# uga-ssrl/SSRLCV

Hardware: AMD Instinct MI355X
Metric: Mpix/s SIFT extract (+ Mmatches/s 128-D brute-force, see `matcher`) (higher is better)
Workload: dtype f32; 1 GPU; 2-view 4096x4096 pair per GPU (tools/scene.py pinhole views (PCG32 terrain + texture through Image::Camera)): SIFT_FeatureFactory::generateFeatures (sparse DoG path) on each image, pixels resident in HBM; images_per_gpu=2, parallelism=image-pair shard, library=release build (libssrlcv_hip_release.so)

## Files before the change

ssrlcv_amd/csrc/dev_switch.h:

```cpp
#pragma once
#include <stddef.h>
#include <stdint.h>
#include <stdlib.h>

#if (defined(SSRLCV_STAMPS) || defined(SSRLCV_MATCH_STATS) || defined(SSRLCV_TIMING_VARIANT)) && !defined(SSRLCV_INSTRUMENTED_BUILD)
#error "SSRLCV_STAMPS / SSRLCV_MATCH_STATS only build through `make instrumented` or the tools/ lab programs (-DSSRLCV_INSTRUMENTED_BUILD)"
#endif
#if defined(SSRLCV_LAB) || defined(SSRLCV_MATCH_LAB) || defined(SSRLCV_LAB_LOCAL_GATHER) || defined(SSRLCV_LAB_UPS_LOADS)
#error "the timing-lab variants (results invalid) were removed in round 6; see git history before 2026-10-05"
#endif

#ifndef SSRLCV_THETAS_LANES_SHIFT
#define SSRLCV_THETAS_LANES_SHIFT 2
#endif
#ifndef SSRLCV_PAIR_F32_MINPX
#define SSRLCV_PAIR_F32_MINPX (~(size_t)0)
#endif
static_assert(SSRLCV_THETAS_LANES_SHIFT >= 0 && SSRLCV_THETAS_LANES_SHIFT <= 2, "k_thetas is built for 1, 2 or 4 lanes per key point");

namespace svdev __attribute__((visibility("hidden"))) {
#ifdef SSRLCV_RELEASE
constexpr bool flag(const char*) { return false; }
constexpr int integer(const char*, int unset) { return unset; }
constexpr size_t size(const char*, size_t unset) { return unset; }
constexpr float real(const char*, float unset) { return unset; }
constexpr char first_char(const char*) { return 0; }
#else
inline const char* env(const char* name) { return getenv(name); }
inline bool flag(const char* name) { return env(name) != nullptr; }
inline int integer(const char* name, int unset) { return env(name) ? atoi(env(name)) : unset; }
inline size_t size(const char* name, size_t unset) { return env(name) ? (size_t)atoll(env(name)) : unset; }
inline float real(const char* name, float unset) { return env(name) ? (float)atof(env(name)) : unset; }
inline char first_char(const char* name) { return env(name) ? env(name)[0] : 0; }
#endif
template <typename T>
constexpr T positive_or(T v, T otherwise) { return v > 0 ? v : otherwise; }
constexpr int one_or_two(int n) { return n == 1 || n == 2 ? n : 0; }
constexpr int lanes_to_shift(int lanes) { return lanes >= 4 ? 2 : (lanes >= 2 ? 1 : 0); }

struct Switches {
  bool gaussValu = flag("SSRLCV_GAUSS_VALU");
  bool gaussMfma = flag("SSRLCV_GAUSS_MFMA");
  bool gaussWide = flag("SSRLCV_GAUSS_WIDE");
  bool gaussNarrow = flag("SSRLCV_GAUSS_NARROW");
  int gaussMfmaMinR = integer("SSRLCV_GAUSS_MFMA_MINR", 11);
  size_t gaussTileMaxPx = size("SSRLCV_GAUSS_TILE_MAXPX", (size_t)1 << 20);
  int gaussRm = integer("SSRLCV_GAUSS_RM", 4 | 8 | 16);
  size_t gaussRmMinPx = size("SSRLCV_GAUSS_RM_MINPX", (size_t)1 << 24);
  int gaussRmOneb = integer("SSRLCV_GAUSS_RM_ONEB", 0);
  int gaussRmRows = integer("SSRLCV_GAUSS_RM_ROWS", 0);
  bool noGaussPair = flag("SSRLCV_NO_GAUSS_PAIR");
  bool noGaussPairRm = flag("SSRLCV_NO_GAUSS_PAIR_RM");
  size_t gaussPairMinPx = size("SSRLCV_GAUSS_PAIR_MINPX", (size_t)1 << 26);
  size_t gaussPairMinPxF32 = size("SSRLCV_GAUSS_PAIR_MINPX_F32", SSRLCV_PAIR_F32_MINPX);
  bool gaussPairValuForm = first_char("SSRLCV_GAUSS_PAIR_FORM") == 'v';
  int pairRows = integer("SSRLCV_PAIR_ROWS", 0);
  bool noUpsampleFusion = flag("SSRLCV_NO_UPSAMPLE_FUSION");
  bool noBinFusion = flag("SSRLCV_NO_BIN_FUSION");
  bool noXcdStrips = flag("SSRLCV_NO_XCD_STRIPS");
  int dogxNpx = integer("SSRLCV_DOGX_NPX", 0);
  int dogSplit = integer("SSRLCV_DOG_SPLIT", 0) != 0 ? 1 : 0;
  unsigned dogxWaves = positive_or((unsigned)integer("SSRLCV_DOGX_WAVES", 0), 14336u);
  int dogx0After = one_or_two(integer("SSRLCV_DOGX0_AFTER", 0));
  bool noOctaveOverlap = flag("SSRLCV_NO_OCTAVE_OVERLAP");
  int octaveOverlapFrom = integer("SSRLCV_OCTAVE_OVERLAP_FROM", 1);
  int phased = integer("SSRLCV_PHASED", 0);
  bool earlyPolar = flag("SSRLCV_EARLY_POLAR");
  bool noEarlyChain = flag("SSRLCV_NO_EARLY_CHAIN");
  bool siftSerial = flag("SSRLCV_SIFT_SERIAL");
  int prio = integer("SSRLCV_PRIO", 0);
  bool sideLowPriority = flag("SSRLCV_SIDE_LOW_PRIORITY");
  int thetasLanesShift = lanes_to_shift(integer("SSRLCV_THETAS_LANES", 1 << SSRLCV_THETAS_LANES_SHIFT));
  bool thetasSplit = flag("SSRLCV_THETAS_SPLIT");
  bool samplingPipelined = flag("SSRLCV_SAMPLING_PIPELINED");
  bool samplingIrregular = flag("SSRLCV_SAMPLING_IRREGULAR");
  bool stagedGlue = (prio & 4) != 0;
#if defined(SSRLCV_INSTRUMENTED_BUILD) && !defined(SSRLCV_RELEASE)
  uint32_t timingThetasSel = env("SSRLCV_TIMING_THETAS_SEL") ? (uint32_t)strtoul(env("SSRLCV_TIMING_THETAS_SEL"), nullptr, 16) : 0xFFFFFu;
#else
  uint32_t timingThetasSel = 0xFFFFFu;
#endif
  bool matchF16 = flag("SSRLCV_MATCH_F16");
  float bandDir = real("SSRLCV_BAND_DIR", 1e30f);
  float bandStrip = real("SSRLCV_BAND_STRIP", 0.0f);
  float bandStripQ = real("SSRLCV_BAND_STRIP_Q", 0.0f);
  int mergeThreads = positive_or(integer("SSRLCV_MERGE_THREADS", 1), 1);
  bool mergeTiming = flag("SSRLCV_MERGE_TIMING");
};

#ifdef SSRLCV_RELEASE
constexpr Switches kDefaults{};
constexpr const Switches& sw() { return kDefaults; }
#else
inline Switches& sw() {
  static Switches s;
  return s;
}
#endif
}
```

ssrlcv_amd/csrc/keypoints.hip:

```cpp
#include <hip/hip_runtime.h>
#include <float.h>
#include <math.h>
#include <stdlib.h>
#include "compact.h"
#include "dev_switch.h"
#include "scan_lookback.h"
#include "device_math.h"
#include "sift_plan.h"
#include "ssrlcv_hip.h"

using svp::OctaveState;

namespace {

struct LevelSet {
  const float* lvl[svp::kGauss];
  const float* lvlMinMax;
  const float* minmax;
  const float2* polar;
  int w, h;
};

struct DogView {
  const float* lo;
// ... 393 lines not shown
        const int lo = st[o].idx[seg], hi = seg < svp::kDog - 1 ? st[o].idx[seg + 1] : st[o].n;
        if (hi > lo) { first = (uint32_t)lo; count = (uint32_t)(hi - lo); }
      }
      tab->first[r] = first;
      tab->count[r] = count;
      tab->start[r] = pos;
      pos += (count + (1u << unitShift) - 1) >> unitShift;
    }
  }
  tab->total = pos;
}
__global__ void k_build_ranges(const OctaveState* st, RangeTable* tab, int unitShift, uint32_t sel) { build_ranges(st, tab, unitShift, sel); }
__global__ void k_book_and_desc_ranges(OctaveState* st, uint32_t* featBase, uint32_t* numFeatures, uint32_t maxFeatures, RangeTable* tab) {
  uint32_t tot = 0;
  for (int o = 0; o < svp::kOctaves; ++o) {
    featBase[o] = tot;
    tot += st[o].hasExtrema ? (uint32_t)st[o].n : 0u;
  }
  if (tot > maxFeatures) tot = maxFeatures;
  *numFeatures = tot;
  build_ranges(st, tab, 0, 0xFFFFFu);
}

constexpr int kOct0Groups = svp::kSampleGroups - 1;
struct GroupCtl {
  uint32_t segStart[svp::kDog];
  uint32_t totals[svp::kSampleGroups + 1];
  uint32_t groupSum[svp::kSampleGroups];
  uint32_t done[svp::kSampleGroups];
  uint32_t regular;
  uint32_t cut[2];
  uint32_t pad[32 - svp::kDog - 3 * svp::kSampleGroups - 4];
};
static_assert(sizeof(GroupCtl) == 128, "four of them + eight range tables fit the plan's 4 KB group block");
__device__ __forceinline__ bool blur_indices_regular(const OctaveState* st) {
  if (!st->hasExtrema) return true;
  bool ok = st->idx[0] == 0;
  for (int k = 1; k < svp::kDog; ++k) ok = ok && st->idx[k - 1] <= st->idx[k];
  return ok && st->idx[svp::kDog - 1] <= st->n;
}
__global__ void k_build_group_ranges(const OctaveState* st, RangeTable* tabs, GroupCtl* ctl, int unitShift, bool forceIrregular) {
  const bool reg = blur_indices_regular(st) && !forceIrregular;
  const uint32_t n0 = st[0].hasExtrema && st[0].n > 0 ? (uint32_t)st[0].n : 0u;
  ctl[0].regular = reg ? 1u : 0u;
  ctl[0].cut[0] = reg && n0 ? (uint32_t)st[0].idx[2] : n0;
  ctl[0].cut[1] = reg && n0 ? (uint32_t)st[0].idx[3] : n0;
  const uint32_t oct0 = 0x1Fu, rest = 0xFFFFFu & ~oct0;
  build_ranges(st, tabs + 0, unitShift, reg ? 0x03u : oct0);
  build_ranges(st, tabs + 1, unitShift, reg ? 0x04u : 0u);
  build_ranges(st, tabs + 2, unitShift, reg ? 0x18u : 0u);
  build_ranges(st, tabs + 3, unitShift, rest);
}
__global__ void k_build_desc_ranges_oct0(const OctaveState* st, RangeTable* tab, const GroupCtl* ctl, int g, uint32_t cap) {
  if (!ctl->regular) {
    build_ranges(st, tab, 0, g == kOct0Groups - 1 ? 0x1Fu : 0u);
    return;
  }
  const int segLo = g == 0 ? 0 : g + 1, segHi = g == 0 ? 2 : (g == 1 ? 3 : svp::kDog);
  const uint32_t end = ctl->totals[g + 1] < cap ? ctl->totals[g + 1] : cap;
  auto start_of = [&](int seg) {
    if (seg >= segHi) return end;
    const uint32_t enc = ctl->segStart[seg];
    const uint32_t v = enc ? enc - 1u : end;
    return v < end ? v : end;
  };
  uint32_t pos = 0;
  for (int k = 0; k < 5; ++k) {
    const int seg = kSegOrder[k];
    for (int o = 0; o < svp::kOctaves; ++o) {
      const int r = k * 4 + o;
      uint32_t first = 0, count = 0;
      if (o == 0 && seg >= segLo && seg < segHi) {
        const uint32_t lo = start_of(seg), hi = start_of(seg + 1);
        if (hi > lo) { first = lo; count = hi - lo; }
      }
      tab->first[r] = first;
      tab->count[r] = count;
      tab->start[r] = pos;
      pos += count;
    }
  }
  tab->total = pos;
}
__device__ __forceinline__ int range_of(const RangeTable* tab, uint32_t u) {
  int r = 0;
#pragma unroll
  for (int k = 1; k < 20; ++k)
    if (tab->start[k] <= u) r = k;
  return r;
}

struct OctaveSet {
  LevelSet L[svp::kOctaves];
  const ssrlcv_sskeypoint* kps[svp::kOctaves];
  float pixelWidth[svp::kOctaves];
  float* thetas[svp::kOctaves];
  uint32_t* thetaCnt[svp::kOctaves];
  const void* consts[svp::kOctaves];
};

template <int MAXO, int LPKS>
__global__ __launch_bounds__(64) void k_thetas(const OctaveState* states, const RangeTable* tab, OctaveSet set, float lambda,
                                               float orientationThreshold) {
  constexpr int LANES = 1 << LPKS, PER_BLOCK = 64 >> LPKS, CW = kThetaChunk * LANES;
  __shared__ float s_hist[36][PER_BLOCK];
  if (blockIdx.x >= tab->total) return;
  const int range = __builtin_amdgcn_readfirstlane(range_of(tab, blockIdx.x));
  const int octave = range & 3, useg = kSegOrder[range >> 2];
  const LevelSet& L = set.L[octave];
  const float pixelWidth = set.pixelWidth[octave];
  const int t = threadIdx.x, sub = t & (LANES - 1), col = t >> LPKS;
  const float fsub2 = (float)(2 * sub);
  const uint32_t local = (blockIdx.x - tab->start[range]) * PER_BLOCK + (uint32_t)(t >> LPKS);
  const bool have = local < tab->count[range];
  const int gi = (int)(tab->first[range] + local);
  const float pi = SSRLCV_PI_F;
  const float rad10 = pi / 18.0f;
  const float inv10 = 1.0f / rad10;
  ssrlcv_sskeypoint kp;
  kp.loc.x = kp.loc.y = 0.0f;
  kp.sigma = 1.0f;
  if (have) kp = set.kps[octave][gi];
  const float kx = kp.loc.x, ky = kp.loc.y;
  const float windowWidth = ceilf(kp.sigma * 3.0f * lambda / pixelWidth);
  const float minx = kx - windowWidth, miny = ky - windowWidth, maxx = kx + windowWidth, maxy = ky + windowWidth;
  const bool inside = have && useg >= 1 && useg <= 3 &&
                      !(minx < 0.0f || miny < 0.0f || maxx >= (unsigned)(L.w - 1) || maxy >= (unsigned)(L.h - 1));
#pragma unroll
  for (int i = 0; i < 36 * PER_BLOCK / 64; ++i) (&s_hist[0][0])[i * 64 + t] = 0.0f;
  const float weight = 2.0f * lambda * lambda * kp.sigma * kp.sigma;
  const float rweight = 1.0f / weight;
  const int W = L.w;
  const size_t levelStride = svp::polar_level_stride(L.w, L.h);
  {
    const float2* base = L.polar + (size_t)(useg - 1) * levelStride;
    const __amdgpu_buffer_rsrc_t rsrc = __builtin_amdgcn_make_buffer_rsrc((void*)base, 0, (int)(uint32_t)(levelStride * 8), 0x00020000);
    typedef unsigned u32x4 __attribute__((ext_vector_type(4)));
    typedef unsigned u32x2 __attribute__((ext_vector_type(2)));
    struct Cursor { float x, y, ty2; unsigned rowoff; bool act; };
    Cursor cf;
    cf.x = minx;
    cf.y = miny;
    cf.ty2 = (miny - ky) * (miny - ky);
    cf.rowoff = (unsigned)round_pos(miny) * (unsigned)W + 1u;
    cf.act = inside;
    auto advance = [&](Cursor& c) {
      float xn = c.x + (float)CW;
      if (__any(c.act && !(c.x >= (float)CW))) {
        float ch = c.x;
#pragma unroll 8
        for (int i = 0; i < CW; ++i) ch += 1.0f;
        xn = c.x >= (float)CW ? xn : ch;
      }
      if (c.act) {
        if (xn <= maxx) {
          c.x = xn;
        } else {
          c.x = minx;
          c.y += 1.0f;
          if (!(c.y <= maxy)) c.act = false;
          const float ty = c.y - ky;
          c.ty2 = ty * ty;
          c.rowoff = (unsigned)round_pos(c.y) * (unsigned)W + 1u;
        }
      }
    };
    typedef u32x4 Chunk[kThetaChunk / 2];
// ... 91 lines not shown
              const float n1 = fmaf(mg[2 * j + 1], wg[2 * j + 1], slot[2 * j + 1] == slot[2 * j] ? n0 : h1);
              *slot[2 * j] = n0;
              *slot[2 * j + 1] = n1;
            }
            if (LANES > 1) __builtin_amdgcn_wave_barrier();
          }
        }
      };
      weigh_half(std::integral_constant<int, 0>{});
      if (upperHalf) weigh_half(std::integral_constant<int, 1>{});
      vote_half(std::integral_constant<int, 0>{});
      if (upperHalf) vote_half(std::integral_constant<int, 1>{});
    };
    while (__any(ca.act)) {
      step(qa, ca, qb, cb);
      if (!__any(cb.act)) break;
      step(qb, cb, qa, ca);
    }
  }
  uint32_t cnt = 0;
  float outTheta[MAXO];
#pragma unroll
  for (int i = 0; i < MAXO; ++i) outTheta[i] = -FLT_MAX;
  if (inside && sub == 0) {
    float maxHist = 0.0f;
    for (int i = 0; i < 36; ++i) {
      const float h = s_hist[i][col];
      if (h > maxHist) maxHist = h;
    }
    maxHist *= orientationThreshold;
    float bestMag[MAXO], bestTh[MAXO];
#pragma unroll
    for (int i = 0; i < MAXO; ++i) { bestMag[i] = 0.0f; bestTh[i] = 0.0f; }
    float hprev = s_hist[35][col], hb = s_hist[0][col];
    for (int b = 0; b < 36; ++b) {
      const float hnext = s_hist[b == 35 ? 0 : b + 1][col];
      if (!(hb < maxHist || hb < hprev || hb < hnext || hb < bestMag[MAXO - 1])) {
        float tmag = hb;
        float tt = (hprev - hnext) / (hprev - (2.0f * hb) + hnext);
        tt *= (pi / 36.0f);
        tt += (b * rad10);
        tt = fmodf(tt + (2.0f * pi), 2.0f * pi);
#pragma unroll
        for (int i = 0; i < MAXO; ++i) {
          if (tmag > bestMag[i]) {
#pragma unroll
            for (int ii = i; ii < MAXO; ++ii) {
              float m2 = bestMag[ii], t2 = bestTh[ii];
              bestMag[ii] = tmag;
              bestTh[ii] = tt;
              tmag = m2;
              tt = t2;
            }
          }
        }
      }
      hprev = hb;
      hb = hnext;
    }
#pragma unroll
    for (int i = 0; i < MAXO; ++i) {
      if (bestMag[i] != 0.0f) { outTheta[i] = bestTh[i]; cnt = i + 1; }
    }
  }
  if (have && sub == 0) {
#pragma unroll
    for (int i = 0; i < MAXO; ++i) set.thetas[octave][(size_t)gi * svp::kMaxOrient + i] = outTheta[i];
    set.thetaCnt[octave][gi] = cnt;
  }
}

__device__ __forceinline__ float uniform_f(float v) {
  return __builtin_bit_cast(float, __builtin_amdgcn_readfirstlane(__builtin_bit_cast(int, v)));
}
struct DescConst {
  float c, s;
  float windowWidth;
  float invExpDen;
  float voteScale;
  float invBin;
  uint32_t magic;
  int32_t segment;
};
static_assert(sizeof(DescConst) == 32, "one s_load_dwordx8");
__global__ __launch_bounds__(256) void k_desc_consts(const RangeTable* tab, OctaveSet set, float lambda, const OctaveState* states,
                                                     const GroupCtl* regularCtl) {
  const uint32_t total = tab->total;
  const bool fromTable = regularCtl != nullptr && regularCtl->regular != 0u;
  for (uint32_t u = blockIdx.x * 256 + threadIdx.x; u < total; u += gridDim.x * 256) {
    const int range = range_of(tab, u);
    const int octave = range & 3;
    const int i = (int)(tab->first[range] + (u - tab->start[range]));
    const ssrlcv_sskeypoint* kps = set.kps[octave];
    const float pixelWidth = set.pixelWidth[octave];
    DescConst* __restrict__ out = (DescConst*)const_cast<void*>(set.consts[octave]);
    DescConst d;
    const float theta = kps[i].theta;
    d.c = sv_cosf(-theta);
    d.s = sv_sinf(-theta);
    d.windowWidth = ceilf(kps[i].sigma * lambda / pixelWidth);
    d.invExpDen = 1.0f / (2.0f * d.windowWidth * d.windowWidth);
    int boundExp;
    (void)frexpf(1.4143f * ((d.windowWidth + 2.0f) * (d.windowWidth + 2.0f)), &boundExp);
    d.voteScale = ldexpf(1.0f, 31 - boundExp);
    d.invBin = 1.0f / (d.windowWidth / 2.0f);
    const unsigned wi = (unsigned)(int)d.windowWidth;
    d.magic = wi > 1u ? 0xFFFFFFFFu / wi + 1u : 0u;
    d.segment = fromTable ? kSegOrder[range >> 2] : segment_of(states + octave, i);
    out[i] = d;
  }
}

__device__ __forceinline__ unsigned vote_u32(float v) {
  int r;
  asm("v_cvt_rpi_i32_f32 %0, %1" : "=v"(r) : "v"(v));
  return (unsigned)r;
}

#ifndef SSRLCV_DESC_COPIES
#define SSRLCV_DESC_COPIES 8
#endif
constexpr int kDescCopies = SSRLCV_DESC_COPIES;
#ifndef SSRLCV_DESC_VGPRS
#define SSRLCV_DESC_VGPRS 64
#endif
__global__ __launch_bounds__(256) __attribute__((amdgpu_waves_per_eu(4, 8), amdgpu_num_vgpr(SSRLCV_DESC_VGPRS), amdgpu_num_sgpr(102))) void k_descriptors(const RangeTable* tab, OctaveSet set, const uint32_t* featBase,
                                                     ssrlcv_sift_feature* __restrict__ features, uint32_t maxFeatures) {
  __shared__ unsigned s_bins[4][(1 + 128 + 2) * kDescCopies];
  __shared__ __attribute__((aligned(8))) uint8_t s_bytes[4][128];
  const int lane = threadIdx.x & 63, wave = __builtin_amdgcn_readfirstlane(threadIdx.x >> 6);
  unsigned* bins = s_bins[wave] + kDescCopies;
  const int copy = lane & (kDescCopies - 1);
  const float pi = SSRLCV_PI_F;
  const float rad45 = pi / 4.0f;
  const float inv45 = 1.0f / rad45;
  const uint32_t totalUnits = tab->total;
  for (uint32_t unit = blockIdx.x * 4 + wave; unit < totalUnits; unit += gridDim.x * 4) {
    const int range = range_of(tab, unit);
    const int octave = range & 3;
    const int gi = (int)(tab->first[range] + (unit - tab->start[range]));
    const LevelSet& L = set.L[octave];
    const float pixelWidth = set.pixelWidth[octave];
    const float2* __restrict__ polar = L.polar;
    const DescConst dc = reinterpret_cast<const DescConst*>(set.consts[octave])[gi];
    const ssrlcv_sskeypoint kp = set.kps[octave][gi];
    const int seg = dc.segment;
    const float kx = kp.loc.x, ky = kp.loc.y;
    const float theta = kp.theta;
    const float windowWidth = dc.windowWidth;
    const float binWidth = windowWidth / 2.0f;
    const float c = dc.c, s = dc.s;
    const float2* __restrict__ pl = polar + (size_t)(seg - 1) * svp::polar_level_stride(L.w, L.h) + 1;
#pragma unroll
    for (int i = 0; i < 2 * kDescCopies; ++i) bins[i * 64 + lane] = 0u;
    f32x2 rc[16];
    {
      const int ci = lane & 15;
      const float hx = ((float)(ci >> 2) * 0.5f - 0.75f) * windowWidth, hy = ((float)(ci & 3) * 0.5f - 0.75f) * windowWidth;
      const float rx = (hx * c) + (hy * s), ry = (-hx * s) + (hy * c);
#pragma unroll
      for (int cell = 0; cell < 16; ++cell) {
        if ((cell >> 2) == 0 || (cell & 3) == 0) continue;
        rc[cell].x = __builtin_bit_cast(float, __builtin_amdgcn_readlane(__builtin_bit_cast(int, rx), cell));
        rc[cell].y = __builtin_bit_cast(float, __builtin_amdgcn_readlane(__builtin_bit_cast(int, ry), cell));
      }
    }
    const float expDen = 2.0f * windowWidth * windowWidth, invExpDen = dc.invExpDen, invBin = dc.invBin;
    const float voteScale = dc.voteScale;
    const int Wi = (int)windowWidth;
    const unsigned centreIdx = (unsigned)(Wi * (Wi + 1));
    const unsigned magic = dc.magic;
    auto sample = [&](unsigned idx, float& cx, float& cy, bool& ok) {
      const unsigned yq = Wi == 1 ? idx : __umulhi(idx, magic);
      const unsigned xq = idx - yq * (unsigned)Wi + 1u;
      const bool centre = idx >= centreIdx;
      const float x = centre ? 0.0f : (float)(int)xq;
      const float y = centre ? 0.0f : (float)(int)yq;
      cx = (x * c) + (y * s);
      cy = (-x * s) + (y * c);
      ok = idx <= centreIdx && fmaxf(fabsf(cx), fabsf(cy)) <= windowWidth;
    };
    auto gather = [&](float px, float py) { return polar_px(pl, L.w, round_coord(px), round_coord(py)); };
    auto split = [&](float2 pg, bool live, float& w0, float& w1, unsigned*& pa, float& ang, bool& odd) {
      ang = fmod_2pi_above(pg.y - theta + (2.0f * pi), 2.0f * pi);
      const float t45 = ang * inv45;
      const float fk = floorf(t45);
      const float u = t45 - fk;
      odd = live && !(u > 1.0e-4f && u < 0.9999f);
      int k0 = (int)fk;
      const float a0 = fabsf(ang - (fk * rad45)), a1 = fabsf(ang - ((fk + 1.0f) * rad45));
      w0 = (live && !odd && (unsigned)k0 < 8u) ? 1.0f - sv::exact_div3(a0, rad45, inv45) : 0.0f;
      w1 = (live && !odd && (unsigned)(k0 + 1) < 8u) ? 1.0f - sv::exact_div3(a1, rad45, inv45) : 0.0f;
      k0 = k0 < -1 ? -1 : k0;
      pa = bins + k0 * kDescCopies + copy;
    };
    float ncx, ncy;
    bool nok;
    sample((unsigned)lane, ncx, ncy, nok);
    float2 npg[4] = {make_float2(0.0f, 0.0f), make_float2(0.0f, 0.0f), make_float2(0.0f, 0.0f), make_float2(0.0f, 0.0f)};
    auto gather4 = [&]() {
      npg[0] = gather(ncx + kx, ncy + ky);
      npg[1] = gather(kx - ncy, ncx + ky);
      npg[2] = gather(kx - ncx, ky - ncy);
      npg[3] = gather(ncy + kx, ky - ncx);
    };
    if (nok) gather4();
    for (unsigned base = 0; base <= centreIdx; base += 64) {
      const float cx = ncx, cy = ncy;
      const bool ok = nok;
      const float2 pg0 = npg[0], pg1 = npg[1], pg2 = npg[2], pg3 = npg[3];
      const bool turned = ok && base + (unsigned)lane < centreIdx;
      sample(base + 64 + (unsigned)lane, ncx, ncy, nok);
      if (nok) gather4();
      const float r2n = -((cx * cx) + (cy * cy));
      const float g = sv::expf_nonpos(sv::exact_div3(r2n, expDen, invExpDen)) * voteScale;
      float a0, a1, b0, b1, c0, c1, d0, d1, angA, angB, angC, angD;
      bool oddA, oddB, oddC, oddD;
      unsigned *pa, *pb, *pc, *pd;
      split(pg0, ok, a0, a1, pa, angA, oddA);
      split(pg1, turned, b0, b1, pb, angB, oddB);
      split(pg2, turned, c0, c1, pc, angC, oddC);
      split(pg3, turned, d0, d1, pd, angD, oddD);
      const float magA = pg0.x * g, magB = pg1.x * g, magC = pg2.x * g, magD = pg3.x * g;
      const float bwl = ok ? binWidth : -1.0f;
#pragma unroll
      for (int cell = 0; cell < 16; ++cell) {
        const int nx = cell >> 2, ny = cell & 3;
        if (nx == 0 || ny == 0) continue;
        const int cellB = (3 - ny) * 4 + nx, cellC = 15 - cell, cellD = ny * 4 + (3 - nx);
        const float tx = fabsf(rc[cell].x - cx), ty = fabsf(rc[cell].y - cy);
        if (fmaxf(tx, ty) <= bwl) {
          const float wxy = (1.0f - sv::exact_div3(tx, binWidth, invBin)) * (1.0f - sv::exact_div3(ty, binWidth, invBin));
          atomicAdd(pa + cell * 8 * kDescCopies, vote_u32((wxy * a0) * magA));
          atomicAdd(pa + cell * 8 * kDescCopies + kDescCopies, vote_u32((wxy * a1) * magA));
          atomicAdd(pb + cellB * 8 * kDescCopies, vote_u32((wxy * b0) * magB));
          atomicAdd(pb + cellB * 8 * kDescCopies + kDescCopies, vote_u32((wxy * b1) * magB));
          atomicAdd(pc + cellC * 8 * kDescCopies, vote_u32((wxy * c0) * magC));
          atomicAdd(pc + cellC * 8 * kDescCopies + kDescCopies, vote_u32((wxy * c1) * magC));
          atomicAdd(pd + cellD * 8 * kDescCopies, vote_u32((wxy * d0) * magD));
          atomicAdd(pd + cellD * 8 * kDescCopies + kDescCopies, vote_u32((wxy * d1) * magD));
        }
      }
      if (__ballot(oddA || oddB || oddC || oddD) != 0ull) {
#pragma unroll 1
        for (int m = 0; m < 4; ++m) {
          const bool odd = m == 0 ? oddA : m == 1 ? oddB : m == 2 ? oddC : oddD;
          if (!odd) continue;
          const float mcx = m == 0 ? cx : m == 1 ? -cy : m == 2 ? -cx : cy;
          const float mcy = m == 0 ? cy : m == 1 ? cx : m == 2 ? -cy : -cx;
          const float mang = m == 0 ? angA : m == 1 ? angB : m == 2 ? angC : angD;
          const float mmag = m == 0 ? magA : m == 1 ? magB : m == 2 ? magC : magD;
#pragma unroll 1
          for (int cell = 0; cell < 16; ++cell) {
            const int ci = lane & 15;
            (void)ci;
            const float hx0 = ((float)(cell >> 2) * 0.5f - 0.75f) * windowWidth, hy0 = ((float)(cell & 3) * 0.5f - 0.75f) * windowWidth;
            const float rx = (hx0 * c) + (hy0 * s), ry = (-hx0 * s) + (hy0 * c);
            float hx = fabsf(rx - mcx), hy = fabsf(ry - mcy);
            if (hx <= binWidth && hy <= binWidth) {
              hx = hx / binWidth;
              hy = hy / binWidth;
              for (int k = 0; k < 8; ++k) {
                float angle = fabsf(mang - ((float)k * rad45));
                if (angle < rad45) {
                  angle /= rad45;
                  const float temp = (1.0f - hx) * (1.0f - hy) * (1.0f - angle) * mmag;
                  atomicAdd(bins + (cell * 8 + k) * kDescCopies + copy, vote_u32(temp));
                }
              }
            }
          }
        }
      }
    }
    __builtin_amdgcn_wave_barrier();
    unsigned t0 = 0u, t1 = 0u;
#pragma unroll
    for (int cpy = 0; cpy < kDescCopies; ++cpy) {
      t0 += bins[lane * kDescCopies + cpy];
      t1 += bins[(lane + 64) * kDescCopies + cpy];
    }
    float v0 = (float)t0, v1 = (float)t1;
    float sq = sqrtf(sv::wave_sum((v0 * v0) + (v1 * v1)));
    v0 = v0 / sq;
    v1 = v1 / sq;
    if (v0 > 0.2f) v0 = 0.2f;
    if (v1 > 0.2f) v1 = 0.2f;
    sq = sqrtf(sv::wave_sum((v0 * v0) + (v1 * v1)));
    {
      int b0 = lane, b1 = lane + 64;
      int o0 = (((b0 >> 3) & 3) * 4 + (b0 >> 5)) * 8 + (b0 & 7);
      int o1 = (((b1 >> 3) & 3) * 4 + (b1 >> 5)) * 8 + (b1 & 7);
      s_bytes[wave][o0] = (uint8_t)roundf(255.0f * v0 / sq);
      s_bytes[wave][o1] = (uint8_t)roundf(255.0f * v1 / sq);
    }
    __builtin_amdgcn_wave_barrier();
    const uint32_t fi = featBase[octave] + (uint32_t)gi;
    if (fi < maxFeatures) {
      ssrlcv_sift_feature* f = features + fi;
      if (lane < 16) *reinterpret_cast<uint2*>(&f->values[lane * 8]) = *reinterpret_cast<const uint2*>(&s_bytes[wave][lane * 8]);
      if (lane == 16) {
        f->parent = -1;
        reinterpret_cast<int*>(f)[1] = 0;
        f->theta = kp.theta;
        f->sigma = kp.sigma;
        f->loc.x = kp.loc.x * pixelWidth;
        f->loc.y = kp.loc.y * pixelWidth;
      }
    }
    __builtin_amdgcn_wave_barrier();
  }
}

LevelSet make_levels(const ssrlcv_sift_plan* plan, char* ws, int o) {
  LevelSet L;
  const svp::OctavePlan& oc = plan->oct[o];
  for (int b = 0; b < svp::kGauss; ++b) L.lvl[b] = (const float*)(ws + plan->off_gauss[o][b]);
  L.lvlMinMax = (const float*)(ws + plan->off_minmax) + (size_t)o * 2 * (svp::kGauss + svp::kDog);
  L.minmax = L.lvlMinMax + 2 * svp::kGauss;
  L.polar = (const float2*)(ws + oc.off_polar);
  L.w = (int)oc.w;
  L.h = (int)oc.h;
  return L;
}

void launch_polar(const ssrlcv_sift_plan* plan, char* ws, hipStream_t st, int oFirst = 0, int oLast = svp::kOctaves - 1) {
  PolarJobs jobs;
  uint32_t pos = 0;
  for (int o = 0; o < svp::kOctaves; ++o) {
    const svp::OctavePlan& oc = plan->oct[o];
    jobs.L[o] = make_levels(plan, ws, o);
    jobs.out[o] = (float2*)(ws + oc.off_polar);
    jobs.start[o] = pos;
    jobs.tilesX[o] = (oc.w + 255) / 256;
    if (o >= oFirst && o <= oLast) pos += jobs.tilesX[o] * ((oc.h + kPolRows - 1) / kPolRows);
  }
  jobs.start[svp::kOctaves] = pos;
  hipLaunchKernelGGL(k_polar, dim3(pos), dim3(256), 0, st, jobs);
}

}
namespace svp {
void launch_polar_octave(const ssrlcv_sift_plan* plan, char* ws, int octave, hipStream_t st) {
  PolarJobs jobs;
  const svp::OctavePlan& oc = plan->oct[octave];
  const uint32_t tilesX = (oc.w + 255) / 256, tiles = tilesX * ((oc.h + kPolRows - 1) / kPolRows);
  for (int o = 0; o < svp::kOctaves; ++o) {
    jobs.L[o] = make_levels(plan, ws, octave);
    jobs.out[o] = (float2*)(ws + oc.off_polar);
    jobs.tilesX[o] = tilesX;
    jobs.start[o] = o <= octave ? 0u : tiles;
  }
  jobs.start[svp::kOctaves] = tiles;
  hipLaunchKernelGGL(k_polar, dim3(tiles), dim3(256), 0, st, jobs);
}
}
namespace {
hipError_t run_discard(OctaveState* st, const ssrlcv_sskeypoint* src, ssrlcv_sskeypoint* dst, uint32_t cap,
                       uint32_t* words, hipStream_t stream) {
  const OctaveState* cst = st;
  auto keyfn = [=] __device__(uint32_t i) -> uint32_t {
    if (!cst->hasExtrema || (int)i >= cst->n) return 0u;
    if (src[i].discard) return 0u;
    return 1u << segment_of(cst, (int)i);
  };
  auto emit = [=] __device__(uint32_t i, int, uint32_t d) { dst[d] = src[i]; };
  uint32_t* totals = nullptr;
  auto post = [=] __device__(const uint32_t* tot) { book_discard(st, tot); };
  return svc::partition<svp::kDog, 8>(cap, keyfn, emit, words, &totals, stream, &st->n, 1u, post);
}

constexpr unsigned kWaveKernelOversubscription = 16;
inline unsigned list_blocks(uint32_t cap) {
  unsigned b = (cap + 255) / 256;
  return b > 1024 ? 1024 : b;
}

}

extern "C" {

int ssrlcv_sift_plan_keypoints(const ssrlcv_sift_plan* plan, void* workspace, int octave, ssrlcv_sskeypoint** list,
                               int** blurIndices_dev) {
  if (!plan || !workspace || octave < 0 || octave >= svp::kOctaves) return SSRLCV_ERR_INVALID_ARG;
  char* ws = (char*)workspace;
  if (list) *list = (ssrlcv_sskeypoint*)(ws + (plan->listInB[octave] ? plan->oct[octave].off_kpB : plan->oct[octave].off_kpA));
  if (blurIndices_dev) *blurIndices_dev = (int*)(ws + plan->off_state + sizeof(OctaveState) * octave);
  return SSRLCV_OK;
}

// ... 415 lines not shown
  }
  return SSRLCV_OK;
}

int stage_orientations(const ssrlcv_sift_plan* plan, char* ws, uint32_t* numFeatures, hipStream_t caller, svp::PlanAsync* as, bool polarDone,
                       bool restInFlight = false, bool prologueDone = false) {
  OctaveState* states = (OctaveState*)(ws + plan->off_state);
  const uint32_t maxO = plan->params.maxOrientations;
  OctaveSet set = make_set(plan, ws);
  RangeTable* thetaRanges = theta_tab(plan, ws, 0);
  const uint32_t thetaSel = svdev::sw().timingThetasSel;
  const int lanesShift = svdev::sw().thetasLanesShift;
  const float lambdaO = plan->params.orientationContribWidth, othr = plan->params.orientationThreshold;
  if (restInFlight) {
    hipLaunchKernelGGL(k_build_ranges, dim3(1), dim3(1), 0, caller, states, thetaRanges, 6 - lanesShift, 0x1Fu & thetaSel);
    launch_thetas(maxO, lanesShift, thetas_grid(plan, 0, 0, lanesShift), caller, (const OctaveState*)states, (const RangeTable*)thetaRanges, set,
                  lambdaO, othr);
    int rc = launch_expand(plan, ws, 0, 0, 1, caller);
    if (rc) return rc;
    plan->listInB[0] ^= 1;
    SSRLCV_HIP_TRY(hipStreamWaitEvent(caller, as->expandJoin[1], 0));
    return SSRLCV_OK;
  }
  if (!svdev::sw().stagedGlue) {
    if (!prologueDone) launch_orient_prologue(plan, ws, caller);
    if (!polarDone) launch_polar(plan, ws, caller);
    launch_thetas(maxO, lanesShift, thetas_grid(plan, 0, svp::kOctaves - 1, lanesShift), caller, (const OctaveState*)states, (const RangeTable*)thetaRanges, set, lambdaO, othr);
    launch_expand_all(plan, ws, numFeatures, caller);
    for (int o = 0; o < svp::kOctaves; ++o) plan->listInB[o] ^= 1;
    return SSRLCV_OK;
  }
  if (!prologueDone) {
    const int rc = orientations_prologue(plan, ws, caller, as);
    if (rc) return rc;
  }
  if (!polarDone) launch_polar(plan, ws, caller);
  launch_thetas(maxO, lanesShift, thetas_grid(plan, 0, svp::kOctaves - 1, lanesShift), caller, (const OctaveState*)states, (const RangeTable*)thetaRanges, set, lambdaO, othr);
  if (as) {
    SSRLCV_HIP_TRY(hipEventRecord(as->groupFork, caller));
    for (int o = 1; o < svp::kOctaves; ++o) SSRLCV_HIP_TRY(hipStreamWaitEvent(expand_stream(as, caller, o), as->groupFork, 0));
  }
  for (int o = 0; o < svp::kOctaves; ++o) {
    int rc = launch_expand(plan, ws, o, 0, 1, expand_stream(as, caller, o), true);
    if (rc) return rc;
    plan->listInB[o] ^= 1;
  }
  if (as) {
    for (int o = 1; o < svp::kOctaves; ++o) {
      SSRLCV_HIP_TRY(hipEventRecord(as->groupExpanded[o - 1], expand_stream(as, caller, o)));
      SSRLCV_HIP_TRY(hipStreamWaitEvent(caller, as->groupExpanded[o - 1], 0));
    }
  }
  return SSRLCV_OK;
}

void book_features(const ssrlcv_sift_plan* plan, char* ws, uint32_t* numFeatures, hipStream_t caller, bool withDescRanges = false) {
  if (withDescRanges)
    hipLaunchKernelGGL(k_book_and_desc_ranges, dim3(1), dim3(1), 0, caller, (OctaveState*)(ws + plan->off_state),
                       (uint32_t*)(ws + plan->oct[0].off_featBase), numFeatures, plan->maxFeatures, desc_tab(plan, ws, 0));
  else
    hipLaunchKernelGGL(k_book_featbase, dim3(1), dim3(1), 0, caller, (OctaveState*)(ws + plan->off_state),
                       (uint32_t*)(ws + plan->oct[0].off_featBase), numFeatures, plan->maxFeatures);
}

unsigned desc_blocks(const ssrlcv_sift_plan* plan, int oFirst, int oLast, unsigned* maxBlocks) {
  unsigned blocks = 0, mx = 1;
  for (int o = oFirst; o <= oLast; ++o) {
    blocks += list_blocks(plan->oct[o].cap);
    mx = list_blocks(plan->oct[o].cap) > mx ? list_blocks(plan->oct[o].cap) : mx;
  }
  if (maxBlocks) *maxBlocks = mx;
  return blocks;
}

int stage_descriptors(const ssrlcv_sift_plan* plan, char* ws, ssrlcv_sift_feature* features, hipStream_t caller, bool rangesBuilt = false) {
  OctaveState* states = (OctaveState*)(ws + plan->off_state);
  OctaveSet set = make_set(plan, ws);
  RangeTable* descRanges = desc_tab(plan, ws, 0);
  uint32_t* featBase = (uint32_t*)(ws + plan->oct[0].off_featBase);
  unsigned maxBlocks = 1;
  const unsigned descBlocks = desc_blocks(plan, 0, svp::kOctaves - 1, &maxBlocks);
  if (!rangesBuilt) hipLaunchKernelGGL(k_build_ranges, dim3(1), dim3(1), 0, caller, states, descRanges, 0, 0xFFFFFu);
  hipLaunchKernelGGL(k_desc_consts, dim3(maxBlocks * svp::kOctaves), dim3(256), 0, caller, (const RangeTable*)descRanges, set,
                     plan->params.descriptorContribWidth, (const OctaveState*)states, (const GroupCtl*)nullptr);
  hipLaunchKernelGGL(k_descriptors, dim3(descBlocks * kWaveKernelOversubscription), dim3(256), 0, caller, (const RangeTable*)descRanges, set,
                     (const uint32_t*)featBase, features, plan->maxFeatures);
  return SSRLCV_OK;
}

int stage_sampling_pipelined(const ssrlcv_sift_plan* plan, char* ws, ssrlcv_sift_feature* features, uint32_t* numFeatures,
                             hipStream_t caller, svp::PlanAsync* as) {
  OctaveState* states = (OctaveState*)(ws + plan->off_state);
  const uint32_t maxO = plan->params.maxOrientations;
  const float lambdaO = plan->params.orientationContribWidth, othr = plan->params.orientationThreshold;
  const float lambdaD = plan->params.descriptorContribWidth;
  uint32_t* featBase = (uint32_t*)(ws + plan->oct[0].off_featBase);
  OctaveSet setT = make_set(plan, ws);
  for (int o = 0; o < svp::kOctaves; ++o) plan->listInB[o] ^= 1;
  OctaveSet setD = make_set(plan, ws);
  for (int o = 0; o < svp::kOctaves; ++o) plan->listInB[o] ^= 1;
  const hipStream_t gs[svp::kSampleGroups] = {caller, as->chain, as->chain2, as->table};
  const int lanesShift = svdev::sw().thetasLanesShift;
  unsigned thetaBlocks[svp::kSampleGroups], descBlocks[svp::kSampleGroups], constBlocks[svp::kSampleGroups];
  for (int g = 0; g < svp::kSampleGroups; ++g) {
    const int oFirst = g < kOct0Groups ? 0 : 1, oLast = g < kOct0Groups ? 0 : svp::kOctaves - 1;
    thetaBlocks[g] = thetas_grid(plan, oFirst, oLast, lanesShift);
    unsigned mx = 1;
    descBlocks[g] = desc_blocks(plan, oFirst, oLast, &mx) * kWaveKernelOversubscription;
    constBlocks[g] = mx * (unsigned)(oLast - oFirst + 1);
  }
  SSRLCV_HIP_TRY(hipMemsetAsync(group_ctl(plan, ws, 0), 0, sizeof(GroupCtl) * svp::kOctaves, caller));
  SSRLCV_HIP_TRY(hipMemsetAsync(featBase, 0, 4 * svp::kOctaves, caller));
  const bool forceIrregular = svdev::sw().samplingIrregular;
  hipLaunchKernelGGL(k_build_group_ranges, dim3(1), dim3(1), 0, caller, (const OctaveState*)states, theta_tab(plan, ws, 0), group_ctl(plan, ws, 0), 6 - lanesShift,
                     forceIrregular);
  SSRLCV_HIP_TRY(hipEventRecord(as->groupFork, caller));
  for (int g = 1; g < svp::kSampleGroups; ++g) SSRLCV_HIP_TRY(hipStreamWaitEvent(gs[g], as->groupFork, 0));
  for (int g = 0; g < svp::kSampleGroups; ++g)
    launch_thetas(maxO, lanesShift, thetaBlocks[g], gs[g], (const OctaveState*)states, (const RangeTable*)theta_tab(plan, ws, g), setT, lambdaO, othr);
  for (int g = 0; g < kOct0Groups; ++g) {
    if (g > 0) SSRLCV_HIP_TRY(hipStreamWaitEvent(gs[g], as->groupExpanded[g - 1], 0));
    int rc = launch_expand(plan, ws, 0, g, kOct0Groups, gs[g]);
    if (rc) return rc;
    SSRLCV_HIP_TRY(hipEventRecord(as->groupExpanded[g], gs[g]));
    hipLaunchKernelGGL(k_build_desc_ranges_oct0, dim3(1), dim3(1), 0, gs[g], (const OctaveState*)states, desc_tab(plan, ws, g),
                       (const GroupCtl*)group_ctl(plan, ws, 0), g, plan->oct[0].cap);
    hipLaunchKernelGGL(k_desc_consts, dim3(constBlocks[g]), dim3(256), 0, gs[g], (const RangeTable*)desc_tab(plan, ws, g), setD, lambdaD,
                       (const OctaveState*)states, (const GroupCtl*)group_ctl(plan, ws, 0));
    if (g > 0) SSRLCV_HIP_TRY(hipEventRecord(as->groupReady[g], gs[g]));
  }
  {
    const int g = svp::kSampleGroups - 1;
    for (int o = 1; o < svp::kOctaves; ++o) {
      int rc = launch_expand(plan, ws, o, 0, 1, gs[g]);
      if (rc) return rc;
    }
    SSRLCV_HIP_TRY(hipStreamWaitEvent(gs[g], as->groupExpanded[kOct0Groups - 1], 0));
    book_features(plan, ws, numFeatures, gs[g]);
    hipLaunchKernelGGL(k_build_ranges, dim3(1), dim3(1), 0, gs[g], (const OctaveState*)states, desc_tab(plan, ws, g), 0, 0xFFFFFu & ~0x1Fu);
    hipLaunchKernelGGL(k_desc_consts, dim3(constBlocks[g]), dim3(256), 0, gs[g], (const RangeTable*)desc_tab(plan, ws, g), setD, lambdaD,
                       (const OctaveState*)states, (const GroupCtl*)nullptr);
    SSRLCV_HIP_TRY(hipEventRecord(as->groupReady[g], gs[g]));
  }
  for (int o = 0; o < svp::kOctaves; ++o) plan->listInB[o] ^= 1;
  for (int g = 0; g < svp::kSampleGroups; ++g) {
    if (g > 0) SSRLCV_HIP_TRY(hipStreamWaitEvent(caller, as->groupReady[g], 0));
    hipLaunchKernelGGL(k_descriptors, dim3(descBlocks[g]), dim3(256), 0, caller, (const RangeTable*)desc_tab(plan, ws, g), setD,
                       (const uint32_t*)featBase, features, plan->maxFeatures);
  }
  return SSRLCV_OK;
}

int run_list_chain(const ssrlcv_sift_plan* plan, char* ws, int o, hipStream_t s) {
  const int stop = plan->stopStage;
  const ListCtx c = make_ctx(plan, ws, o, s);
  int rc = stage_extrema(c, stop >= 1);
  if (!rc && stop >= 2) rc = stage_refine(c);
  if (!rc && stop >= 5) rc = stage_noise_edges_window(c);
  else {
    if (!rc && stop >= 3) rc = stage_noise(c, svp::kNoiseThreshold);
    if (!rc && stop >= 4) rc = stage_edges(c);
  }
  return rc;
}

}
namespace svp {
int launch_chain_octave(const ssrlcv_sift_plan* plan, char* ws, int octave, hipStream_t st) { return run_list_chain(plan, ws, octave, st); }
}
extern "C" {

static void drain_side_streams(const ssrlcv_sift_plan* plan, hipStream_t st) {
  svp::PlanAsync* as = plan->asyncState == 1 ? plan->async : nullptr;
  if (as) {
    for (hipStream_t side : {as->chain, as->table, as->chain2, as->polar}) {
      if (hipEventRecord(as->fork, side) == hipSuccess) (void)hipStreamWaitEvent(st, as->fork, 0);
    }
    (void)hipGetLastError();
  }
  plan->chain0InFlight = 0;
  plan->polarInFlight = 0;
}
static int describe_impl(const ssrlcv_sift_plan* plan, void* workspace, ssrlcv_sift_feature* features, uint32_t* numFeatures, ssrlcv_stream_t stream);
int ssrlcv_hip_sift_describe(const ssrlcv_sift_plan* plan, void* workspace, ssrlcv_sift_feature* features, uint32_t* numFeatures,
                             ssrlcv_stream_t stream) {
  const int rc = describe_impl(plan, workspace, features, numFeatures, stream);
  if (rc && plan) drain_side_streams(plan, (hipStream_t)stream);
  return rc;
}
static int describe_impl(const ssrlcv_sift_plan* plan, void* workspace, ssrlcv_sift_feature* features,
                             uint32_t* numFeatures, ssrlcv_stream_t stream) {
  if (!plan || !workspace || !numFeatures) return SSRLCV_ERR_INVALID_ARG;
  char* ws = (char*)workspace;
  const int stop = plan->stopStage;
  if (stop >= 7 && !features) return SSRLCV_ERR_INVALID_ARG;
  svp::PlanAsync* as = svp::plan_async(plan);
  const hipStream_t caller = (hipStream_t)stream;
  const bool splitWanted = svdev::sw().thetasSplit, pipelinedSampling = svdev::sw().samplingPipelined;
  const bool splitRest = as && stop >= 6 && !plan->polarInFlight && splitWanted && !pipelinedSampling;
  if (splitRest) SSRLCV_HIP_TRY(hipMemsetAsync(group_ctl(plan, ws, 0), 0, sizeof(GroupCtl) * svp::kOctaves, caller));
  const bool pipelinedFits = stop >= 7 && as && pipelinedSampling && expand_scratch_fits(plan, 0, kOct0Groups);
  const bool glue = stop >= 6 && !svdev::sw().stagedGlue && !splitRest && !pipelinedFits;
  const bool callerFree = as && glue && (plan->chain0InFlight & 1);
  const bool tablesOnCaller = callerFree && !plan->polarInFlight && !(svdev::sw().prio & 1);
  if (as) {
    SSRLCV_HIP_TRY(hipEventRecord(as->fork, caller));
    SSRLCV_HIP_TRY(hipStreamWaitEvent(as->chain, as->fork, 0));
    SSRLCV_HIP_TRY(hipStreamWaitEvent(as->chain2, as->fork, 0));
    SSRLCV_HIP_TRY(hipStreamWaitEvent(as->table, as->fork, 0));
    if ((svdev::sw().prio & 1)) SSRLCV_HIP_TRY(hipStreamWaitEvent(as->polar, as->fork, 0));
    if (tablesOnCaller) {
      launch_polar(plan, ws, caller);
    } else if (stop >= 6 && !plan->polarInFlight) {
      const hipStream_t ps = (svdev::sw().prio & 1) ? as->polar : as->table;
      if (splitRest) {
        launch_polar(plan, ws, ps, 1, svp::kOctaves - 1);
        SSRLCV_HIP_TRY(hipEventRecord(as->polarDone[1], ps));
        launch_polar(plan, ws, ps, 0, 0);
      } else {
        launch_polar(plan, ws, ps);
      }
    }
  }
  for (int o = 0; o < svp::kOctaves; ++o) {
// ... 478 lines not shown
```

Before: 3629 Mpix/s.

## Pair descriptor histogram cells by orientation class to skip redundant window tests

k_desc_consts now classifies each keypoint by its rotation (c,s) into one of two classes and packs that class bit into the segment word. k_descriptors uses the class to visit the nine inner cells as four disjoint pairs plus the centre cell, assuming at most one cell of each pair is hit in the common case. This cuts the unrolled per-sample test-and-vote loop over cells and the divergent atomic branches. Constant and keypoint data are also read through the scalar constant address space, and the occupancy hint is raised to 8 waves per EU. Vote order changes and a tighter register budget may cause spills.

```diff
diff --git a/ssrlcv_amd/csrc/dev_switch.h b/ssrlcv_amd/csrc/dev_switch.h
--- a/ssrlcv_amd/csrc/dev_switch.h
+++ b/ssrlcv_amd/csrc/dev_switch.h
@@ -75,6 +75,7 @@
   bool samplingPipelined = flag("SSRLCV_SAMPLING_PIPELINED");
   bool samplingIrregular = flag("SSRLCV_SAMPLING_IRREGULAR");
   bool stagedGlue = (prio & 4) != 0;
+  int descPairClass = (prio & 8) != 0 ? 1 : ((prio & 16) != 0 ? 2 : 0);
 #if defined(SSRLCV_INSTRUMENTED_BUILD) && !defined(SSRLCV_RELEASE)
   uint32_t timingThetasSel = env("SSRLCV_TIMING_THETAS_SEL") ? (uint32_t)strtoul(env("SSRLCV_TIMING_THETAS_SEL"), nullptr, 16) : 0xFFFFFu;
 #else
diff --git a/ssrlcv_amd/csrc/keypoints.hip b/ssrlcv_amd/csrc/keypoints.hip
--- a/ssrlcv_amd/csrc/keypoints.hip
+++ b/ssrlcv_amd/csrc/keypoints.hip
@@ -499,7 +499,8 @@
   }
   tab->total = pos;
 }
-__device__ __forceinline__ int range_of(const RangeTable* tab, uint32_t u) {
+template <typename Table>
+__device__ __forceinline__ int range_of(Table tab, uint32_t u) {
   int r = 0;
 #pragma unroll
   for (int k = 1; k < 20; ++k)
@@ -757,9 +758,10 @@
   uint32_t magic;
   int32_t segment;
 };
+constexpr int kDescClassBit = 8;
 static_assert(sizeof(DescConst) == 32, "one s_load_dwordx8");
 __global__ __launch_bounds__(256) void k_desc_consts(const RangeTable* tab, OctaveSet set, float lambda, const OctaveState* states,
-                                                     const GroupCtl* regularCtl) {
+                                                     const GroupCtl* regularCtl, int forceClass) {
   const uint32_t total = tab->total;
   const bool fromTable = regularCtl != nullptr && regularCtl->regular != 0u;
   for (uint32_t u = blockIdx.x * 256 + threadIdx.x; u < total; u += gridDim.x * 256) {
@@ -781,7 +783,10 @@
     d.invBin = 1.0f / (d.windowWidth / 2.0f);
     const unsigned wi = (unsigned)(int)d.windowWidth;
     d.magic = wi > 1u ? 0xFFFFFFFFu / wi + 1u : 0u;
-    d.segment = fromTable ? kSegOrder[range >> 2] : segment_of(states + octave, i);
+    const float nA = fmaxf(fabsf((2.0f * d.c) + d.s), fabsf(d.c - (2.0f * d.s)));
+    const float nB = fmaxf(fabsf(d.c + (2.0f * d.s)), fabsf((2.0f * d.c) - d.s));
+    const bool classB = forceClass != 0 ? forceClass == 2 : !(nA >= nB);
+    d.segment = (fromTable ? kSegOrder[range >> 2] : segment_of(states + octave, i)) | ((int)classB << kDescClassBit);
     out[i] = d;
   }
 }
@@ -799,7 +804,7 @@
 #ifndef SSRLCV_DESC_VGPRS
 #define SSRLCV_DESC_VGPRS 64
 #endif
-__global__ __launch_bounds__(256) __attribute__((amdgpu_waves_per_eu(4, 8), amdgpu_num_vgpr(SSRLCV_DESC_VGPRS), amdgpu_num_sgpr(102))) void k_descriptors(const RangeTable* tab, OctaveSet set, const uint32_t* featBase,
+__global__ __launch_bounds__(256) __attribute__((amdgpu_waves_per_eu(8, 8), amdgpu_num_vgpr(SSRLCV_DESC_VGPRS), amdgpu_num_sgpr(102))) void k_descriptors(const RangeTable* tab, OctaveSet set, const uint32_t* featBase,
                                                      ssrlcv_sift_feature* __restrict__ features, uint32_t maxFeatures) {
   __shared__ unsigned s_bins[4][(1 + 128 + 2) * kDescCopies];
   __shared__ __attribute__((aligned(8))) uint8_t s_bytes[4][128];
@@ -809,22 +814,28 @@
   const float pi = SSRLCV_PI_F;
   const float rad45 = pi / 4.0f;
   const float inv45 = 1.0f / rad45;
-  const uint32_t totalUnits = tab->total;
+  typedef const __attribute__((address_space(4))) RangeTable* ConstTable;
+  typedef const __attribute__((address_space(4))) DescConst* ConstDesc;
+  typedef const __attribute__((address_space(4))) ssrlcv_sskeypoint* ConstKp;
+  const ConstTable ctab = (ConstTable)tab;
+  const uint32_t totalUnits = ctab->total;
   for (uint32_t unit = blockIdx.x * 4 + wave; unit < totalUnits; unit += gridDim.x * 4) {
-    const int range = range_of(tab, unit);
+    const int range = range_of(ctab, unit);
     const int octave = range & 3;
-    const int gi = (int)(tab->first[range] + (unit - tab->start[range]));
+    const int gi = (int)(ctab->first[range] + (unit - ctab->start[range]));
     const LevelSet& L = set.L[octave];
     const float pixelWidth = set.pixelWidth[octave];
     const float2* __restrict__ polar = L.polar;
-    const DescConst dc = reinterpret_cast<const DescConst*>(set.consts[octave])[gi];
-    const ssrlcv_sskeypoint kp = set.kps[octave][gi];
-    const int seg = dc.segment;
-    const float kx = kp.loc.x, ky = kp.loc.y;
-    const float theta = kp.theta;
-    const float windowWidth = dc.windowWidth;
+    const ConstDesc dc = (ConstDesc)set.consts[octave] + gi;
+    const ConstKp kp = (ConstKp)set.kps[octave] + gi;
+    const int segWord = dc->segment;
+    const int seg = segWord & ((1 << kDescClassBit) - 1);
+    const bool classB = (segWord >> kDescClassBit) != 0;
+    const float kx = kp->loc.x, ky = kp->loc.y;
+    const float theta = kp->theta;
+    const float windowWidth = dc->windowWidth;
     const float binWidth = windowWidth / 2.0f;
-    const float c = dc.c, s = dc.s;
+    const float c = dc->c, s = dc->s;
     const float2* __restrict__ pl = polar + (size_t)(seg - 1) * svp::polar_level_stride(L.w, L.h) + 1;
 #pragma unroll
     for (int i = 0; i < 2 * kDescCopies; ++i) bins[i * 64 + lane] = 0u;
@@ -840,11 +851,11 @@
         rc[cell].y = __builtin_bit_cast(float, __builtin_amdgcn_readlane(__builtin_bit_cast(int, ry), cell));
       }
     }
-    const float expDen = 2.0f * windowWidth * windowWidth, invExpDen = dc.invExpDen, invBin = dc.invBin;
-    const float voteScale = dc.voteScale;
+    const float expDen = 2.0f * windowWidth * windowWidth, invExpDen = dc->invExpDen, invBin = dc->invBin;
+    const float voteScale = dc->voteScale;
     const int Wi = (int)windowWidth;
     const unsigned centreIdx = (unsigned)(Wi * (Wi + 1));
-    const unsigned magic = dc.magic;
+    const unsigned magic = dc->magic;
     auto sample = [&](unsigned idx, float& cx, float& cy, bool& ok) {
       const unsigned yq = Wi == 1 ? idx : __umulhi(idx, magic);
       const unsigned xq = idx - yq * (unsigned)Wi + 1u;
@@ -898,23 +909,51 @@
       split(pg3, turned, d0, d1, pd, angD, oddD);
       const float magA = pg0.x * g, magB = pg1.x * g, magC = pg2.x * g, magD = pg3.x * g;
       const float bwl = ok ? binWidth : -1.0f;
-#pragma unroll
-      for (int cell = 0; cell < 16; ++cell) {
-        const int nx = cell >> 2, ny = cell & 3;
-        if (nx == 0 || ny == 0) continue;
-        const int cellB = (3 - ny) * 4 + nx, cellC = 15 - cell, cellD = ny * 4 + (3 - nx);
-        const float tx = fabsf(rc[cell].x - cx), ty = fabsf(rc[cell].y - cy);
-        if (fmaxf(tx, ty) <= bwl) {
-          const float wxy = (1.0f - sv::exact_div3(tx, binWidth, invBin)) * (1.0f - sv::exact_div3(ty, binWidth, invBin));
-          atomicAdd(pa + cell * 8 * kDescCopies, vote_u32((wxy * a0) * magA));
-          atomicAdd(pa + cell * 8 * kDescCopies + kDescCopies, vote_u32((wxy * a1) * magA));
-          atomicAdd(pb + cellB * 8 * kDescCopies, vote_u32((wxy * b0) * magB));
-          atomicAdd(pb + cellB * 8 * kDescCopies + kDescCopies, vote_u32((wxy * b1) * magB));
-          atomicAdd(pc + cellC * 8 * kDescCopies, vote_u32((wxy * c0) * magC));
-          atomicAdd(pc + cellC * 8 * kDescCopies + kDescCopies, vote_u32((wxy * c1) * magC));
-          atomicAdd(pd + cellD * 8 * kDescCopies, vote_u32((wxy * d0) * magD));
-          atomicAdd(pd + cellD * 8 * kDescCopies + kDescCopies, vote_u32((wxy * d1) * magD));
+      constexpr int kCellWords = 8 * kDescCopies;
+      auto cell_test = [&](int cell, float& tx, float& ty) {
+        tx = fabsf(rc[cell].x - cx);
+        ty = fabsf(rc[cell].y - cy);
+        return fmaxf(tx, ty) <= bwl;
+      };
+      auto vote = [&](float tx, float ty, unsigned* qa, unsigned* qb, unsigned* qc, unsigned* qd) {
+        const float wxy = (1.0f - sv::exact_div3(tx, binWidth, invBin)) * (1.0f - sv::exact_div3(ty, binWidth, invBin));
+        atomicAdd(qa, vote_u32((wxy * a0) * magA));
+        atomicAdd(qa + kDescCopies, vote_u32((wxy * a1) * magA));
+        atomicAdd(qb, vote_u32((wxy * b0) * magB));
+        atomicAdd(qb + kDescCopies, vote_u32((wxy * b1) * magB));
+        atomicAdd(qc, vote_u32((wxy * c0) * magC));
+        atomicAdd(qc + kDescCopies, vote_u32((wxy * c1) * magC));
+        atomicAdd(qd, vote_u32((wxy * d0) * magD));
+        atomicAdd(qd + kDescCopies, vote_u32((wxy * d1) * magD));
+      };
+      auto turned_cell = [](int cell) { return (3 - (cell & 3)) * 4 + (cell >> 2); };
+      auto vote_cell = [&](int cell, float tx, float ty) {
+        const int cellB = turned_cell(cell);
+        vote(tx, ty, pa + cell * kCellWords, pb + cellB * kCellWords, pc + (15 - cell) * kCellWords, pd + (15 - cellB) * kCellWords);
+      };
+      auto vote_pair = [&](int cellP, int cellQ) {
+        float txP, tyP, txQ, tyQ;
+        const bool passP = cell_test(cellP, txP, tyP), passQ = cell_test(cellQ, txQ, tyQ);
+        if (passP || passQ) {
+          const int oA = (passP ? cellP : cellQ) * kCellWords, oB = (passP ? turned_cell(cellP) : turned_cell(cellQ)) * kCellWords;
+          vote(passP ? txP : txQ, passP ? tyP : tyQ, pa + oA, pb + oB, (pc + 15 * kCellWords) - oA, (pd + 15 * kCellWords) - oB);
         }
+        if (passP && passQ) vote_cell(cellQ, txQ, tyQ);
+      };
+      if (!classB) {
+        vote_pair(5, 14);
+        vote_pair(6, 15);
+        vote_pair(7, 9);
+        vote_pair(11, 13);
+      } else {
+        vote_pair(5, 11);
+        vote_pair(9, 15);
+        vote_pair(6, 13);
+        vote_pair(7, 14);
+      }
+      {
+        float tx, ty;
+        if (cell_test(10, tx, ty)) vote_cell(10, tx, ty);
       }
       if (__ballot(oddA || oddB || oddC || oddD) != 0ull) {
 #pragma unroll 1
@@ -970,17 +1009,17 @@
       s_bytes[wave][o1] = (uint8_t)roundf(255.0f * v1 / sq);
     }
     __builtin_amdgcn_wave_barrier();
-    const uint32_t fi = featBase[octave] + (uint32_t)gi;
+    const uint32_t fi = ((const __attribute__((address_space(4))) uint32_t*)featBase)[octave] + (uint32_t)gi;
     if (fi < maxFeatures) {
       ssrlcv_sift_feature* f = features + fi;
       if (lane < 16) *reinterpret_cast<uint2*>(&f->values[lane * 8]) = *reinterpret_cast<const uint2*>(&s_bytes[wave][lane * 8]);
       if (lane == 16) {
         f->parent = -1;
         reinterpret_cast<int*>(f)[1] = 0;
-        f->theta = kp.theta;
-        f->sigma = kp.sigma;
-        f->loc.x = kp.loc.x * pixelWidth;
-        f->loc.y = kp.loc.y * pixelWidth;
+        f->theta = kp->theta;
+        f->sigma = kp->sigma;
+        f->loc.x = kp->loc.x * pixelWidth;
+        f->loc.y = kp->loc.y * pixelWidth;
       }
     }
     __builtin_amdgcn_wave_barrier();
@@ -1562,7 +1601,7 @@
   const unsigned descBlocks = desc_blocks(plan, 0, svp::kOctaves - 1, &maxBlocks);
   if (!rangesBuilt) hipLaunchKernelGGL(k_build_ranges, dim3(1), dim3(1), 0, caller, states, descRanges, 0, 0xFFFFFu);
   hipLaunchKernelGGL(k_desc_consts, dim3(maxBlocks * svp::kOctaves), dim3(256), 0, caller, (const RangeTable*)descRanges, set,
-                     plan->params.descriptorContribWidth, (const OctaveState*)states, (const GroupCtl*)nullptr);
+                     plan->params.descriptorContribWidth, (const OctaveState*)states, (const GroupCtl*)nullptr, svdev::sw().descPairClass);
   hipLaunchKernelGGL(k_descriptors, dim3(descBlocks * kWaveKernelOversubscription), dim3(256), 0, caller, (const RangeTable*)descRanges, set,
                      (const uint32_t*)featBase, features, plan->maxFeatures);
   return SSRLCV_OK;
@@ -1606,7 +1645,7 @@
     hipLaunchKernelGGL(k_build_desc_ranges_oct0, dim3(1), dim3(1), 0, gs[g], (const OctaveState*)states, desc_tab(plan, ws, g),
                        (const GroupCtl*)group_ctl(plan, ws, 0), g, plan->oct[0].cap);
     hipLaunchKernelGGL(k_desc_consts, dim3(constBlocks[g]), dim3(256), 0, gs[g], (const RangeTable*)desc_tab(plan, ws, g), setD, lambdaD,
-                       (const OctaveState*)states, (const GroupCtl*)group_ctl(plan, ws, 0));
+                       (const OctaveState*)states, (const GroupCtl*)group_ctl(plan, ws, 0), svdev::sw().descPairClass);
     if (g > 0) SSRLCV_HIP_TRY(hipEventRecord(as->groupReady[g], gs[g]));
   }
   {
@@ -1619,7 +1658,7 @@
     book_features(plan, ws, numFeatures, gs[g]);
     hipLaunchKernelGGL(k_build_ranges, dim3(1), dim3(1), 0, gs[g], (const OctaveState*)states, desc_tab(plan, ws, g), 0, 0xFFFFFu & ~0x1Fu);
     hipLaunchKernelGGL(k_desc_consts, dim3(constBlocks[g]), dim3(256), 0, gs[g], (const RangeTable*)desc_tab(plan, ws, g), setD, lambdaD,
-                       (const OctaveState*)states, (const GroupCtl*)nullptr);
+                       (const OctaveState*)states, (const GroupCtl*)nullptr, svdev::sw().descPairClass);
     SSRLCV_HIP_TRY(hipEventRecord(as->groupReady[g], gs[g]));
   }
   for (int o = 0; o < svp::kOctaves; ++o) plan->listInB[o] ^= 1;
```

Result: no change. 3624 Mpix/s (-0.1%).
